# bliunlpr/Robust_e2e_gan

Measured on NVIDIA B200. Metric: utterances/sec (joint step fwd/bwd), higher is better.
Workload: dtype fp32

## Files before the change

robust_e2e_gan_b200/csrc/attloc_loop.cu:

```cuda
#include <math_constants.h>

#include "attloc_common.cuh"
#include "tc_common.cuh"

namespace re2e {
namespace {

#ifdef RE2E_ATT_DEBUG
__device__ long long g_loop_dbg[2][16 * 512];
#define LOOP_DBG_DECL                                                  \
  __shared__ long long dbg_acc[16];                                    \
  if (threadIdx.x == 0)                                                \
    for (int i_ = 0; i_ < 16; ++i_) dbg_acc[i_] = 0;                   \
  long long dbg_last = clock64()
#define LOOP_MARK(slot)                                              \
  do {                                                               \
    if (threadIdx.x == 0) {                                          \
      const long long t_ = clock64();                                \
      dbg_acc[slot] += t_ - dbg_last;                                \
      dbg_last = t_;                                                 \
    }                                                                \
  } while (0)
#define LOOP_DBG_FLUSH(which)                                                                   \
  do {                                                                                          \
    if (threadIdx.x == 0)                                                                       \
      for (int i_ = 0; i_ < 16; ++i_) g_loop_dbg[which][blockIdx.x * 16 + i_] = dbg_acc[i_];    \
  } while (0)
#else
#define LOOP_DBG_DECL
#define LOOP_MARK(slot)
#define LOOP_DBG_FLUSH(which)
#endif

__device__ __forceinline__ void cp_async4(void *dst_smem, const void *src_gmem) {
  asm volatile("cp.async.ca.shared.global [%0], [%1], 4;" ::"r"(smem_u32(dst_smem)), "l"(src_gmem) : "memory");
}
__device__ __forceinline__ void cp_async_commit() { asm volatile("cp.async.commit_group;" ::: "memory"); }
__device__ __forceinline__ void cp_async_wait_all() { asm volatile("cp.async.wait_group 0;" ::: "memory"); }

__device__ __forceinline__ void warp_reduce10(float (&v)[10], int lane) {
  {
    const bool up = lane & 16;
#pragma unroll
    for (int i = 0; i < 5; ++i) {
      const float send = up ? v[i] : v[i + 5], keep = up ? v[i + 5] : v[i];
      v[i] = keep + __shfl_xor_sync(0xffffffffu, send, 16);
    }
  }
  {
    const bool up = lane & 8;
#pragma unroll
    for (int i = 0; i < 2; ++i) {
      const float send = up ? v[i] : v[i + 3], keep = up ? v[i + 3] : v[i];
      v[i] = keep + __shfl_xor_sync(0xffffffffu, send, 8);
    }
    v[2] += __shfl_xor_sync(0xffffffffu, v[2], 8);
  }
  {
    const bool up = lane & 4;
    const float send = up ? v[0] : v[1], keep = up ? v[1] : v[0];
    v[0] = keep + __shfl_xor_sync(0xffffffffu, send, 4);
    v[2] += __shfl_xor_sync(0xffffffffu, v[2], 4);
  }
  {
    const bool up = lane & 2;
    const float send = up ? v[0] : v[2], keep = up ? v[2] : v[0];
    v[0] = keep + __shfl_xor_sync(0xffffffffu, send, 2);
  }
  v[0] += __shfl_xor_sync(0xffffffffu, v[0], 1);
}

constexpr int kLP = 8;
constexpr int kLW = 2 * kLP;
constexpr int kLT = kLW * 32;
constexpr int kLMaxCL = 8;
constexpr int kKG = 12;

struct LoopGeom {
  int tloc_max, App, CKp, Thp, Dp;
  int col_enc, ncols;
};

struct LoopFwdParams {
  const float *pre, *enc, *dec_proj, *att_init, *W_att, *W_conv, *gvec, *gvec_b;
  float scaling;
  float *c_all, *w_all, *conv_all;
  int S, B, Th, D, A, C, K;
  LoopGeom g;
};

struct LoopBwdParams {
  const float *pre, *enc, *dec_proj, *att_init, *w_all, *conv_all, *dc_all, *dw_all, *W_att, *W_conv, *gvec;
  float scaling;
  float *d_pre, *d_decproj, *acc_slots;
  int slot_stride;
  int S, B, Th, D, A, C, K;
  LoopGeom g;
};

template <int APL, int CP, int DPL>
__global__ void __launch_bounds__(kLT, 1) attloc_loop_fwd_kernel(const LoopFwdParams p) {
  constexpr int NT = kLT;
  constexpr int WP = CP + 1;
  constexpr int CPP = (CP + 3) & ~3;
  extern __shared__ __align__(128) unsigned char smraw[];
  const LoopGeom g = p.g;
  const int C = CP == 10 ? 10 : p.C;
  const int Th = p.Th, D = p.D, A = p.A, K = p.K, S = p.S, B = p.B, filts = (p.K - 1) / 2;
  const int tid = threadIdx.x, lane = tid & 31, warp = tid >> 5, half = warp & 1, pair = warp >> 1;
  const int CL = (int)cluster_nctarank(), rank = (int)cluster_ctarank();
  const int b = blockIdx.x / CL;
  const int t0 = min(Th, rank * g.tloc_max), t1 = min(Th, t0 + g.tloc_max), tloc = t1 - t0;
  const int nch = (tloc + kLP - 1) / kLP;
  const int Dp = g.Dp, Dh = (D + 1) / 2;

  uint64_t *full = reinterpret_cast<uint64_t *>(smraw);
  uint64_t *xbar = full + 1;
  uint64_t *tbar = xbar + 2;
  float *tile = reinterpret_cast<float *>(smraw + 128);
  float *app = tile + (size_t)g.tloc_max * (A + D);
  float *wc_s = app + g.App;
  float *watt_s = wc_s + g.CKp;
  float *convp = watt_s + A * WP;
  float *conv_s = convp + round4(kKQ * g.tloc_max * CP);
  float *e_all = conv_s + g.tloc_max * CPP;
  float *epart = e_all + 2 * g.Thp;
  float *cred = epart + round4(2 * g.tloc_max);
  float *cbuf = cred + kLP * Dp;

  const uint32_t xbytes = (uint32_t)Th * 4u + (rank == 0 ? (uint32_t)CL * (uint32_t)D * 4u : 0u);
  if (tid == 0) {
    mbar_init(full, 1);
    mbar_init(&xbar[0], 1);
    mbar_init(&xbar[1], 1);
    mbar_init(tbar, 1);
    mbar_fence_init();
    mbar_expect_tx(&xbar[0], xbytes);
    mbar_expect_tx(&xbar[1], xbytes);
    if (rank == 0) mbar_expect_tx(tbar, (uint32_t)CL * (uint32_t)D * 4u);
  }
  cluster_arrive_relaxed();
  float gv[APL];
#pragma unroll
  for (int j = 0; j < APL; ++j) gv[j] = __ldg(p.gvec + half * (A / 2) + lane + 32 * j);
  const float gb = __ldg(p.gvec_b);
  for (int i = tid; i < C * K; i += NT) wc_s[i] = __ldg(p.W_conv + i);
  for (int i = tid; i < A * C; i += NT) { const int a = i / C; watt_s[a * WP + (i - a * C)] = __ldg(p.W_att + i); }
  pdl_wait();
  if (tid == 0 && tloc > 0) {
    mbar_expect_tx(full, (uint32_t)tloc * (uint32_t)(A + D) * 4u);
    bulk_g2s(tile, p.pre + ((size_t)b * Th + t0) * A, (uint32_t)tloc * A * 4u, full);
    bulk_g2s(tile + (size_t)g.tloc_max * A, p.enc + ((size_t)b * Th + t0) * D, (uint32_t)tloc * D * 4u, full);
  }
  for (int i = tid; i < g.App; i += NT) {
    const int t = i - filts;
    app[i] = (t >= 0 && t < Th) ? __ldg(p.att_init + (size_t)b * Th + t) : 0.0f;
  }
  __syncthreads();
  constexpr int APH = (APL + 1) / 2;
  float2 WattP[APH][CP];
#pragma unroll
  for (int jp = 0; jp < APH; ++jp) {
    const int a0 = half * (A / 2) + lane + 32 * (2 * jp), a1 = a0 + 32;
#pragma unroll
    for (int c = 0; c < CP; ++c)
      WattP[jp][c] = make_float2(c < C ? watt_s[a0 * WP + c] : 0.0f, (c < C && 2 * jp + 1 < APL) ? watt_s[a1 * WP + c] : 0.0f);
  }
  uint32_t dmask = 0;
#pragma unroll
  for (int j = 0; j < DPL; ++j)
    if (lane + 32 * j < Dh && half * Dh + lane + 32 * j < D) dmask |= 1u << j;
  const int aoff = half * (A / 2) + lane;
  cluster_wait();
  if (tloc > 0) mbar_wait(full, 0);
  LOOP_DBG_DECL;
  LOOP_MARK(0);

  for (int s = 0; s < S; ++s) {
    const uint32_t par = (uint32_t)s & 1u, ph = ((uint32_t)s >> 1) & 1u;
    float *e_cur = e_all + par * g.Thp;
    float *cb = cbuf + par * kLMaxCL * Dp;
    float dp[APL];
#pragma unroll
    for (int j = 0; j < APL; ++j) dp[j] = __ldg(p.dec_proj + ((size_t)s * B + b) * A + aoff + 32 * j);

    {
      const int ntg = (tloc + kTG - 1) / kTG;
      const int Kq = (K + kKQ - 1) / kKQ;
      const int nitems = ntg * C * kKQ;
      for (int item = tid; item < nitems; item += NT) {
        const int tg = item % ntg, rest = item / ntg, c = rest % C, kq = rest / C;
        const int k0 = kq * Kq, k1 = min(K, k0 + Kq);
        const float *wr = wc_s + c * K;
        const float *ar = app + t0 + kTG * tg;
        float a0 = 0.f, a1 = 0.f, a2 = 0.f, a3 = 0.f, a4 = 0.f;
        float x0 = ar[k0], x1 = ar[k0 + 1], x2 = ar[k0 + 2], x3 = ar[k0 + 3];
#pragma unroll 5
        for (int k = k0; k < k1; ++k) {
          const float x4 = ar[k + 4], wv2 = wr[k];
          a0 = fmaf(wv2, x0, a0); a1 = fmaf(wv2, x1, a1); a2 = fmaf(wv2, x2, a2);
          a3 = fmaf(wv2, x3, a3); a4 = fmaf(wv2, x4, a4);
          x0 = x1; x1 = x2; x2 = x3; x3 = x4;
        }
        float *o = convp + ((size_t)kq * g.tloc_max + kTG * tg) * CP + c;
        const int nv = min(kTG, tloc - kTG * tg);
        o[0] = a0;
        if (nv > 1) o[CP] = a1;
        if (nv > 2) o[2 * CP] = a2;
        if (nv > 3) o[3 * CP] = a3;
        if (nv > 4) o[4 * CP] = a4;
      }
    }
    __syncthreads();
    LOOP_MARK(1);
    for (int i = tid; i < tloc * CPP; i += NT) {
      const int tl = i / CPP, c = i - tl * CPP;
      float v = 0.0f;
      if (c < C) {
#pragma unroll
        for (int kq = 0; kq < kKQ; ++kq) v += convp[((size_t)kq * g.tloc_max + tl) * CP + c];
        if (p.conv_all) p.conv_all[(((size_t)s * B + b) * Th + t0 + tl) * C + c] = v;
      }
      conv_s[i] = v;
    }
    __syncthreads();
    LOOP_MARK(2);

    float acc[DPL];
#pragma unroll
    for (int j = 0; j < DPL; ++j) acc[j] = 0.0f;
#pragma unroll 2
    for (int q = 0; q < nch; ++q) {
      const int tl = kLP * q + pair;
      if (tl < tloc) {
        const float *cvp = conv_s + tl * CPP;
        float cv[CPP];
#pragma unroll
        for (int c4 = 0; c4 < CPP; c4 += 4) {
          const float4 t4 = *reinterpret_cast<const float4 *>(cvp + c4);
          cv[c4] = t4.x; cv[c4 + 1] = t4.y; cv[c4 + 2] = t4.z; cv[c4 + 3] = t4.w;
        }
        const float *row = tile + (size_t)tl * A + aoff;
        const float pw = app[filts + t0 + tl];
        const float *er = tile + (size_t)g.tloc_max * A + (size_t)tl * D + half * Dh + lane;
        float part = 0.0f;
#pragma unroll
        for (int jp = 0; jp < APH; ++jp) {
          const bool two = 2 * jp + 1 < APL;
          float2 u = make_float2(dp[2 * jp] + row[64 * jp], two ? dp[2 * jp + 1] + row[64 * jp + 32] : 0.0f);
#pragma unroll
          for (int c = 0; c < CP; ++c) u = __ffma2_rn(WattP[jp][c], make_float2(cv[c], cv[c]), u);
          part = fmaf(gv[2 * jp], tanh_ex2(u.x), part);
          if (two) part = fmaf(gv[2 * jp + 1], tanh_ex2(u.y), part);
        }
#pragma unroll
        for (int j = 0; j < DPL; ++j)
          if (dmask & (1u << j)) acc[j] = fmaf(pw, er[32 * j], acc[j]);
        part = warp_sum(part);
        if (lane == 0) epart[2 * tl + half] = part;
      }
    }
#pragma unroll
    for (int j = 0; j < DPL; ++j)
      if (dmask & (1u << j)) cred[pair * Dp + half * Dh + lane + 32 * j] = acc[j];
    LOOP_MARK(3);
    __syncthreads();
    LOOP_MARK(4);

    for (int d = tid; d < D; d += NT) {
      float sum = 0.0f;
#pragma unroll
      for (int pr = 0; pr < kLP; ++pr) sum += cred[pr * Dp + d];
      st_async_f32(dsmem_addr(cb + rank * Dp + d, 0u), s > 0 ? sum : 0.0f, dsmem_addr(&xbar[par], 0u));
    }
    for (int i = tid; i < tloc * CL; i += NT) {
      const int r = i / tloc, tl = i - r * tloc;
      const float e = p.scaling * ((epart[2 * tl] + epart[2 * tl + 1]) + gb);
      st_async_f32(dsmem_addr(e_cur + t0 + tl, (uint32_t)r), e, dsmem_addr(&xbar[par], (uint32_t)r));
    }
    LOOP_MARK(5);
    mbar_wait(&xbar[par], ph);
    LOOP_MARK(6);
    float M = -CUDART_INF_F;
    for (int t = lane; t < Th; t += 32) M = fmaxf(M, e_cur[t]);
    M = warp_max(M);
    float Ssum = 0.0f;
    for (int t = lane; t < Th; t += 32) Ssum += __expf(e_cur[t] - M);
    Ssum = warp_sum(Ssum);
    const float inv = 1.0f / Ssum;
    for (int t = tid; t < Th; t += NT) {
      const float w = __expf(e_cur[t] - M) * inv;
      app[filts + t] = w;
      if (t >= t0 && t < t1) p.w_all[((size_t)s * B + b) * Th + t] = w;
    }
    if (rank == 0 && s > 0) {
      for (int d = tid; d < D; d += NT) {
        float sum = 0.0f;
        for (int r = 0; r < CL; ++r) sum += cb[r * Dp + d];
        p.c_all[((size_t)(s - 1) * B + b) * D + d] = sum;
      }
    }
    if (tid == 0) mbar_expect_tx(&xbar[par], xbytes);
    __syncthreads();
    LOOP_MARK(7);
  }
  {
    float acc[DPL];
#pragma unroll
    for (int j = 0; j < DPL; ++j) acc[j] = 0.0f;
    for (int q = 0; q < nch; ++q) {
      const int tl = kLP * q + pair;
      if (tl < tloc) {
        const float pw = app[filts + t0 + tl];
        const float *er = tile + (size_t)g.tloc_max * A + (size_t)tl * D + half * Dh + lane;
#pragma unroll
        for (int j = 0; j < DPL; ++j)
          if (dmask & (1u << j)) acc[j] = fmaf(pw, er[32 * j], acc[j]);
      }
    }
#pragma unroll
    for (int j = 0; j < DPL; ++j)
      if (dmask & (1u << j)) cred[pair * Dp + half * Dh + lane + 32 * j] = acc[j];
    __syncthreads();
    float *cb = cbuf + ((uint32_t)S & 1u) * kLMaxCL * Dp;
    for (int d = tid; d < D; d += NT) {
      float sum = 0.0f;
#pragma unroll
      for (int pr = 0; pr < kLP; ++pr) sum += cred[pr * Dp + d];
      st_async_f32(dsmem_addr(cb + rank * Dp + d, 0u), sum, dsmem_addr(tbar, 0u));
    }
    if (rank == 0) {
      mbar_wait(tbar, 0);
      for (int d = tid; d < D; d += NT) {
        float sum = 0.0f;
        for (int r = 0; r < CL; ++r) sum += cb[r * Dp + d];
        p.c_all[((size_t)(S - 1) * B + b) * D + d] = sum;
      }
    }
  }
  LOOP_DBG_FLUSH(0);
}

template <int N>
__device__ __forceinline__ void tmem_ldn(uint32_t taddr, float *v);
template <>
__device__ __forceinline__ void tmem_ldn<1>(uint32_t taddr, float *v) {
  uint32_t r0;
  asm volatile("tcgen05.ld.sync.aligned.32x32b.x1.b32 {%0}, [%1];" : "=r"(r0) : "r"(taddr));
  v[0] = __uint_as_float(r0);
}
template <>
__device__ __forceinline__ void tmem_ldn<2>(uint32_t taddr, float *v) {
  uint32_t r0, r1;
  asm volatile("tcgen05.ld.sync.aligned.32x32b.x2.b32 {%0, %1}, [%2];" : "=r"(r0), "=r"(r1) : "r"(taddr));
  v[0] = __uint_as_float(r0); v[1] = __uint_as_float(r1);
}
template <>
__device__ __forceinline__ void tmem_ldn<4>(uint32_t taddr, float *v) {
  uint32_t r0, r1, r2, r3;
  asm volatile("tcgen05.ld.sync.aligned.32x32b.x4.b32 {%0, %1, %2, %3}, [%4];"
               : "=r"(r0), "=r"(r1), "=r"(r2), "=r"(r3) : "r"(taddr));
  v[0] = __uint_as_float(r0); v[1] = __uint_as_float(r1); v[2] = __uint_as_float(r2); v[3] = __uint_as_float(r3);
}
template <>
__device__ __forceinline__ void tmem_ldn<8>(uint32_t taddr, float *v) {
  uint32_t r[8];
  asm volatile("tcgen05.ld.sync.aligned.32x32b.x8.b32 {%0, %1, %2, %3, %4, %5, %6, %7}, [%8];"
               : "=r"(r[0]), "=r"(r[1]), "=r"(r[2]), "=r"(r[3]), "=r"(r[4]), "=r"(r[5]), "=r"(r[6]), "=r"(r[7])
               : "r"(taddr));
#pragma unroll
  for (int i = 0; i < 8; ++i) v[i] = __uint_as_float(r[i]);
}
template <int N>
__device__ __forceinline__ void tmem_stn(uint32_t taddr, const float *v);
template <>
__device__ __forceinline__ void tmem_stn<1>(uint32_t taddr, const float *v) {
  asm volatile("tcgen05.st.sync.aligned.32x32b.x1.b32 [%0], {%1};" ::"r"(taddr), "r"(__float_as_uint(v[0])) : "memory");
}
template <>
__device__ __forceinline__ void tmem_stn<2>(uint32_t taddr, const float *v) {
  asm volatile("tcgen05.st.sync.aligned.32x32b.x2.b32 [%0], {%1, %2};" ::"r"(taddr), "r"(__float_as_uint(v[0])),
               "r"(__float_as_uint(v[1]))
               : "memory");
}
template <>
__device__ __forceinline__ void tmem_stn<4>(uint32_t taddr, const float *v) {
  asm volatile("tcgen05.st.sync.aligned.32x32b.x4.b32 [%0], {%1, %2, %3, %4};" ::"r"(taddr),
               "r"(__float_as_uint(v[0])), "r"(__float_as_uint(v[1])), "r"(__float_as_uint(v[2])),
               "r"(__float_as_uint(v[3]))
               : "memory");
}
template <>
__device__ __forceinline__ void tmem_stn<8>(uint32_t taddr, const float *v) {
  asm volatile("tcgen05.st.sync.aligned.32x32b.x8.b32 [%0], {%1, %2, %3, %4, %5, %6, %7, %8};" ::"r"(taddr),
               "r"(__float_as_uint(v[0])), "r"(__float_as_uint(v[1])), "r"(__float_as_uint(v[2])),
               "r"(__float_as_uint(v[3])), "r"(__float_as_uint(v[4])), "r"(__float_as_uint(v[5])),
               "r"(__float_as_uint(v[6])), "r"(__float_as_uint(v[7]))
               : "memory");
}
__device__ __forceinline__ void tmem_wait_ld() { asm volatile("tcgen05.wait::ld.sync.aligned;" ::: "memory"); }
__device__ __forceinline__ void tmem_wait_st() { asm volatile("tcgen05.wait::st.sync.aligned;" ::: "memory"); }
template <int N>
__device__ __forceinline__ void tmem_load(uint32_t taddr, float *v) {
  if constexpr (N >= 8) { tmem_ldn<8>(taddr, v); if constexpr (N > 8) tmem_load<N - 8>(taddr + 8, v + 8); }
  else if constexpr (N >= 4) { tmem_ldn<4>(taddr, v); if constexpr (N > 4) tmem_load<N - 4>(taddr + 4, v + 4); }
  else if constexpr (N >= 2) { tmem_ldn<2>(taddr, v); if constexpr (N > 2) tmem_load<N - 2>(taddr + 2, v + 2); }
  else { tmem_ldn<1>(taddr, v); }
}
template <int N>
__device__ __forceinline__ void tmem_store(uint32_t taddr, const float *v) {
  if constexpr (N >= 8) { tmem_stn<8>(taddr, v); if constexpr (N > 8) tmem_store<N - 8>(taddr + 8, v + 8); }
  else if constexpr (N >= 4) { tmem_stn<4>(taddr, v); if constexpr (N > 4) tmem_store<N - 4>(taddr + 4, v + 4); }
  else if constexpr (N >= 2) { tmem_stn<2>(taddr, v); if constexpr (N > 2) tmem_store<N - 2>(taddr + 2, v + 2); }
  else { tmem_stn<1>(taddr, v); }
}

template <int APL, int CP, int DPL2>
__global__ void __launch_bounds__(kLT, 1) attloc_loop_bwd_kernel(const LoopBwdParams p) {
  constexpr int NT = kLT;
  constexpr int WP = CP + 1;
  constexpr int CPP = (CP + 3) & ~3;
  constexpr int CH2 = (CP + 1) / 2;
  extern __shared__ __align__(128) unsigned char smraw[];
  const LoopGeom g = p.g;
  const int C = CP == 10 ? 10 : p.C;
  const int Th = p.Th, D = p.D, A = p.A, K = p.K, S = p.S, B = p.B, filts = (p.K - 1) / 2;
  const int tid = threadIdx.x, lane = tid & 31, warp = tid >> 5, half = warp & 1, pair = warp >> 1;
  const int CL = (int)cluster_nctarank(), rank = (int)cluster_ctarank();
  const int b = blockIdx.x / CL;
  const int t0 = min(Th, rank * g.tloc_max), t1 = min(Th, t0 + g.tloc_max), tloc = t1 - t0;
  const int nchx = (tloc + kLP - 1) / kLP;
  const int nche = (tloc + kLW - 1) / kLW;
  const int nchx_max = (g.tloc_max + kLP - 1) / kLP, nche_max = (g.tloc_max + kLW - 1) / kLW;

  uint64_t *done_x = reinterpret_cast<uint64_t *>(smraw);
  uint64_t *xbar1 = done_x + 1;
  uint64_t *xbar2 = xbar1 + 2;
  uint32_t *tmem_slot = reinterpret_cast<uint32_t *>(xbar2 + 2);
  float *xs = reinterpret_cast<float *>(smraw + 128);
  float *dcvT = xs + (size_t)g.tloc_max * A;
  float *app = dcvT + 2 * CP * g.App;
  float *wc_s = app + g.App;
  float *conv_s = wc_s + g.CKp;
  float *w_s = conv_s + g.tloc_max * CPP;
  float *dwt_s = w_s + round4(g.tloc_max);
  float *de_s = dwt_s + round4(g.tloc_max);
  float *dwn_s = de_s + round4(g.tloc_max);
  float *dcv_p = dwn_s + round4(g.tloc_max);
  float *ddp_w = dcv_p + 2 * g.tloc_max * 16;
  float *scr = ddp_w + kLW * (A / 2);
  float *ddp_x = scr + max(A * WP, round4(kKQ * CP * g.tloc_max));
  float *xch = ddp_x + 2 * kLMaxCL * A;
  float *slot = p.acc_slots + (size_t)blockIdx.x * p.slot_stride;

  const uint32_t x1bytes = (uint32_t)CL * 4u;
  const uint32_t x2bytes = (uint32_t)Th * (uint32_t)C * 4u + (rank == 0 ? (uint32_t)CL * (uint32_t)A * 4u : 0u);
  if (tid == 0) {
    mbar_init(done_x, kLW);
    for (int i = 0; i < 2; ++i) { mbar_init(&xbar1[i], 1); mbar_init(&xbar2[i], 1); }
    mbar_fence_init();
    for (int i = 0; i < 2; ++i) { mbar_expect_tx(&xbar1[i], x1bytes); mbar_expect_tx(&xbar2[i], x2bytes); }
  }
  cluster_arrive_relaxed();
  if (warp == 0) tmem_alloc(tmem_slot, 512);
  float gv[APL];
#pragma unroll
  for (int j = 0; j < APL; ++j) gv[j] = __ldg(p.gvec + half * (A / 2) + lane + 32 * j);
  for (int i = tid; i < C * K; i += NT) wc_s[i] = __ldg(p.W_conv + i);
  for (int i = tid; i < A * C; i += NT) { const int a = i / C; scr[a * WP + (i - a * C)] = __ldg(p.W_att + i); }
  {
    const int padn = g.App - Th;
    for (int i = tid; i < 2 * CP * padn; i += NT) {
      const int c = i / padn, o = i - c * padn;
      dcvT[c * g.App + (o < filts ? o : Th + o)] = 0.0f;
    }
    for (int i = tid; i < g.tloc_max * CPP; i += NT) conv_s[i] = 0.0f;
    for (int i = tid; i < round4(g.tloc_max); i += NT) dwn_s[i] = 0.0f;
  }
  tc_fence_before();
  __syncthreads();
  tc_fence_after();
  const uint32_t tbase = *tmem_slot + ((uint32_t)(32 * (warp & 3)) << 16);
  const uint32_t tcol_pre = tbase + (uint32_t)((warp >> 2) * nchx_max * APL);
  const uint32_t tcol_enc = tbase + (uint32_t)(g.col_enc + (warp >> 2) * nche_max * DPL2);
  float2 WattC[APL][CH2];
#pragma unroll
  for (int j = 0; j < APL; ++j) {
    const int a = half * (A / 2) + lane + 32 * j;
#pragma unroll
    for (int c2 = 0; c2 < CH2; ++c2)
      WattC[j][c2] = make_float2(2 * c2 < C ? scr[a * WP + 2 * c2] : 0.0f, 2 * c2 + 1 < C ? scr[a * WP + 2 * c2 + 1] : 0.0f);
  }
  const int aoff = half * (A / 2) + lane;
  pdl_wait();
  for (int q = 0; q < nchx; ++q) {
    const int tl = kLP * q + pair;
    float v[APL];
#pragma unroll
    for (int j = 0; j < APL; ++j) v[j] = tl < tloc ? __ldg(p.pre + ((size_t)b * Th + t0 + tl) * A + aoff + 32 * j) : 0.0f;
    tmem_store<APL>(tcol_pre + (uint32_t)(q * APL), v);
  }
  for (int q = 0; q < nche; ++q) {
    const int tl = kLW * q + warp;
    float v[DPL2];
#pragma unroll
    for (int j = 0; j < DPL2; ++j)
      v[j] = (tl < tloc && lane + 32 * j < D) ? __ldg(p.enc + ((size_t)b * Th + t0 + tl) * D + lane + 32 * j) : 0.0f;
    tmem_store<DPL2>(tcol_enc + (uint32_t)(q * DPL2), v);
  }
  tmem_wait_st();
  __syncthreads();
  cluster_wait();

  float pacc[kKG];
#pragma unroll
  for (int i = 0; i < kKG; ++i) pacc[i] = 0.0f;
  float dgv[APL];
#pragma unroll
  for (int j = 0; j < APL; ++j) dgv[j] = 0.0f;
  float dgb = 0.0f;
  const int nkg = (K + kKG - 1) / kKG;
  const bool conv_thread = tid >= A && tid - A < C * nkg;
  const int cw_c = conv_thread ? (tid - A) / nkg : 0, cw_kb = conv_thread ? ((tid - A) % nkg) * kKG : 0;
  LOOP_DBG_DECL;
  LOOP_MARK(0);

  for (int it = 0; it < S; ++it) {
    const int s = S - 1 - it;
    const uint32_t par = (uint32_t)it & 1u, ph = ((uint32_t)it >> 1) & 1u;
    float *dcv_cur = dcvT + par * CP * g.App;
    float *ddpx = ddp_x + par * kLMaxCL * A;
    float *xc = xch + par * kLMaxCL;
    const size_t sb = (size_t)s * B + b;
    float dcr[DPL2];
#pragma unroll
    for (int j = 0; j < DPL2; ++j) dcr[j] = (p.dc_all && lane + 32 * j < D) ? __ldg(p.dc_all + sb * D + lane + 32 * j) : 0.0f;
    float dp[APL];
#pragma unroll
    for (int j = 0; j < APL; ++j) dp[j] = __ldg(p.dec_proj + sb * A + aoff + 32 * j);
    for (int i = tid; i < tloc; i += NT) {
      w_s[i] = __ldg(p.w_all + sb * Th + t0 + i);
      dwt_s[i] = dwn_s[i] + (p.dw_all ? __ldg(p.dw_all + sb * Th + t0 + i) : 0.0f);
    }
    for (int i = tid; i < tloc * C; i += NT) {
      const int tl = i / C;
      conv_s[tl * CPP + (i - tl * C)] = __ldg(p.conv_all + (sb * Th + t0) * C + i);
    }
    {
      const float *prev = s == 0 ? p.att_init + (size_t)b * Th : p.w_all + (sb - B) * Th;
      for (int i = tid; i < g.App; i += NT) {
        const int t = i - filts;
        app[i] = (t >= 0 && t < Th) ? __ldg(prev + t) : 0.0f;
      }
    }
    __syncthreads();
    LOOP_MARK(1);

    for (int q = 0; q < nche; ++q) {
      const int tl = kLW * q + warp;
      float ev[DPL2];
      tmem_load<DPL2>(tcol_enc + (uint32_t)(q * DPL2), ev);
      tmem_wait_ld();
      float dot = 0.0f;
#pragma unroll
      for (int j = 0; j < DPL2; ++j) dot = fmaf(dcr[j], ev[j], dot);
      dot = warp_sum(dot);
      if (lane == 0 && tl < tloc) dwt_s[tl] += dot;
    }
    __syncthreads();
    LOOP_MARK(2);
    if (warp == 0) {
      float s1 = 0.0f;
      for (int tl = lane; tl < tloc; tl += 32) s1 = fmaf(w_s[tl], dwt_s[tl], s1);
      s1 = warp_sum(s1);
      if (lane < CL) st_async_f32(dsmem_addr(xc + rank, (uint32_t)lane), s1, dsmem_addr(&xbar1[par], (uint32_t)lane));
    }
    mbar_wait(&xbar1[par], ph);
    float Stot = 0.0f;
    for (int r = 0; r < CL; ++r) Stot += xc[r];
    for (int tl = tid; tl < tloc; tl += NT) de_s[tl] = p.scaling * w_s[tl] * (dwt_s[tl] - Stot);
    if (tid == 0) {
      mbar_expect_tx(&xbar1[par], x1bytes);
      if (it > 0) bulk_wait<0>();
    }
    __syncthreads();
    LOOP_MARK(3);

    float ddp[APL];
#pragma unroll
    for (int j = 0; j < APL; ++j) ddp[j] = 0.0f;
    float pn[APL];
    tmem_load<APL>(tcol_pre, pn);
#pragma unroll 1
    for (int q = 0; q < nchx; ++q) {
      const int tl = kLP * q + pair;
      tmem_wait_ld();
      float pv[APL];
#pragma unroll
      for (int j = 0; j < APL; ++j) {
        asm volatile("" : "+f"(pn[j]));
        pv[j] = pn[j];
      }
      if (q + 1 < nchx) tmem_load<APL>(tcol_pre + (uint32_t)((q + 1) * APL), pn);
      if (tl < tloc) {
        const float de = de_s[tl];
        const float *cvp = conv_s + tl * CPP;
        float cv[CPP];
#pragma unroll
        for (int c4 = 0; c4 < CPP; c4 += 4) {
          const float4 t4 = *reinterpret_cast<const float4 *>(cvp + c4);
          cv[c4] = t4.x; cv[c4 + 1] = t4.y; cv[c4 + 2] = t4.z; cv[c4 + 3] = t4.w;
        }
        float2 dcv2[8];
#pragma unroll
        for (int c = 0; c < 8; ++c) dcv2[c] = make_float2(0.0f, 0.0f);
        float *row = xs + (size_t)tl * A + aoff;
#pragma unroll
        for (int j = 0; j < APL; ++j) {
          float2 u2 = make_float2(pv[j] + dp[j], 0.0f);
#pragma unroll
          for (int c2 = 0; c2 < CH2; ++c2)
            u2 = __ffma2_rn(WattC[j][c2], make_float2(cv[2 * c2], 2 * c2 + 1 < CPP ? cv[2 * c2 + 1] : 0.0f), u2);
          const float x = tanh_ex2(u2.x + u2.y);
          dgv[j] = fmaf(de, x, dgv[j]);
          const float dt = de * gv[j] * (1.0f - x * x);
          ddp[j] += dt;
          row[32 * j] = dt;
          const float2 dt2 = make_float2(dt, dt);
#pragma unroll
          for (int c2 = 0; c2 < CH2; ++c2) dcv2[c2] = __ffma2_rn(dt2, WattC[j][c2], dcv2[c2]);
        }
        if constexpr (CP == 10) {
          float dcv[10];
#pragma unroll
          for (int c = 0; c < 5; ++c) { dcv[2 * c] = dcv2[c].x; dcv[2 * c + 1] = dcv2[c].y; }
          warp_reduce10(dcv, lane);
          if ((lane & 1) == 0 && ((lane & 2) == 0 || (lane & 12) == 0)) {
            const int b4 = (lane >> 4) & 1, b3 = (lane >> 3) & 1, b2 = (lane >> 2) & 1;
            const int ci = 5 * b4 + ((lane & 2) ? 2 : (b2 ? (b3 ? 4 : 1) : (b3 ? 3 : 0)));
            dcv_p[(half * g.tloc_max + tl) * 16 + ci] = dcv[0];
          }
        } else {
          float dcv[16];
#pragma unroll
          for (int c = 0; c < 8; ++c) { dcv[2 * c] = dcv2[c].x; dcv[2 * c + 1] = dcv2[c].y; }
          warp_reduce16(dcv, lane);
          if ((lane & 1) == 0) {
            const int ci = ((lane >> 4) & 1) * 8 + ((lane >> 3) & 1) * 4 + ((lane >> 2) & 1) * 2 + ((lane >> 1) & 1);
            dcv_p[(half * g.tloc_max + tl) * 16 + ci] = dcv[0];
          }
// ... 91 lines not shown
#pragma unroll 5
        for (int k = k0; k < k1; ++k) {
          const float x0 = dr[-k], wv = wr[k];
          a0 = fmaf(wv, x0, a0); a1 = fmaf(wv, x1, a1); a2 = fmaf(wv, x2, a2);
          a3 = fmaf(wv, x3, a3); a4 = fmaf(wv, x4, a4);
          x4 = x3; x3 = x2; x2 = x1; x1 = x0;
        }
        float *o = scr + ((size_t)(kq * C + c)) * g.tloc_max + kTG * sg;
        const int nv = min(kTG, tloc - kTG * sg);
        o[0] = a0;
        if (nv > 1) o[1] = a1;
        if (nv > 2) o[2] = a2;
        if (nv > 3) o[3] = a3;
        if (nv > 4) o[4] = a4;
      }
    }
    if (tid == 0) mbar_expect_tx(&xbar2[par], x2bytes);
    __syncthreads();
    LOOP_MARK(9);
    if (s > 0) {
      for (int tl = tid; tl < tloc; tl += NT) {
        float sum = 0.0f;
        for (int i = 0; i < kKQ * C; ++i) sum += scr[(size_t)i * g.tloc_max + tl];
        dwn_s[tl] = sum;
      }
    }
    LOOP_MARK(10);
  }

  LOOP_DBG_FLUSH(1);
  if (tid < A) {
#pragma unroll
    for (int c = 0; c < CP; ++c)
      if (c < C) slot[tid * C + c] = pacc[c];
  } else if (conv_thread) {
#pragma unroll
    for (int i = 0; i < kKG; ++i)
      if (cw_kb + i < K) slot[A * C + cw_c * K + cw_kb + i] = pacc[i];
  }
  __syncthreads();
#pragma unroll
  for (int j = 0; j < APL; ++j) ddp_w[warp * (A / 2) + lane + 32 * j] = dgv[j];
  __syncthreads();
  for (int a = tid; a < A; a += NT) {
    const int h = a >= A / 2 ? 1 : 0, ai = a - h * (A / 2);
    float sg = 0.0f;
#pragma unroll
    for (int pr = 0; pr < kLP; ++pr) sg += ddp_w[(2 * pr + h) * (A / 2) + ai];
    slot[A * C + C * K + a] = sg;
  }
  if (warp == kLW - 1 && lane == 0) slot[A * C + C * K + A] = dgb;
  if (tid == 0) bulk_wait<0>();
  tc_fence_before();
  __syncthreads();
  if (warp == 0) tmem_dealloc(*tmem_slot, 512);
}

inline int loop_check_dims(int S, int B, int Th, int D, int A, int C, int K) {
  if (S <= 0 || B <= 0 || Th <= 0 || D <= 0 || A <= 0 || C <= 0 || K <= 0) return RE2E_E_ARG;
  if ((K & 1) == 0) return RE2E_E_ARG;
  if (A % 64 != 0 || A > 512 || (D & 3) || D > 512 || C > 16) return RE2E_E_UNSUPPORTED;
  const int apl = A / 64;
  if (!(apl == 1 || apl == 2 || apl == 4 || apl == 5 || apl == 8)) return RE2E_E_UNSUPPORTED;
  return RE2E_OK;
}

inline int pick_cl(int B, int Th) {
  const int sms = num_sms();
  int CL = 1;
  while (CL < kLMaxCL && B * CL * 2 <= sms) CL *= 2;
  while (CL > 1 && (Th + CL - 1) / CL < kLP) CL /= 2;
  return CL;
}

inline void loop_geom_common(int Th, int D, int C, int K, int CL, LoopGeom &g) {
  const int filts = (K - 1) / 2;
  g.tloc_max = (Th + CL - 1) / CL;
  g.App = round4(Th + 2 * filts + 8);
  g.CKp = round4(C * K);
  g.Thp = round4(Th);
  g.Dp = round4(D);
  g.col_enc = 0;
  g.ncols = 0;
}

inline bool loop_geom_fwd(int B, int Th, int D, int A, int C, int K, int CP, int &CL, LoopGeom &g, size_t &smem) {
  CL = pick_cl(B, Th);
  const int CPP = round4(CP);
  for (;;) {
    loop_geom_common(Th, D, C, K, CL, g);
    const size_t floats = (size_t)g.tloc_max * (A + D) + g.App + g.CKp + (size_t)A * (CP + 1) +
                          round4(kKQ * g.tloc_max * CP) + (size_t)g.tloc_max * CPP + 2 * (size_t)g.Thp +
                          round4(g.tloc_max) + round4(2 * g.tloc_max) + 2 * kLW + (size_t)kLP * g.Dp +
                          2 * (size_t)kLMaxCL * g.Dp + 4 * kLMaxCL;
    smem = 128 + sizeof(float) * floats;
    if (smem <= 226 * 1024) return true;
    if (CL >= kLMaxCL || B * CL * 2 > num_sms()) return false;
    CL *= 2;
  }
}

inline bool loop_geom_bwd(int B, int Th, int D, int A, int C, int K, int CP, int dpl2, int &CL, LoopGeom &g,
                          size_t &smem) {
  CL = pick_cl(B, Th);
  const int CPP = round4(CP);
  const int nkg = (K + kKG - 1) / kKG;
  if (A + C * nkg > kLT) return false;
  for (;;) {
    loop_geom_common(Th, D, C, K, CL, g);
    const int nchx_max = (g.tloc_max + kLP - 1) / kLP, nche_max = (g.tloc_max + kLW - 1) / kLW;
    g.col_enc = 4 * nchx_max * (A / 64);
    g.ncols = g.col_enc + 4 * nche_max * dpl2;
    const size_t scr = (size_t)A * (CP + 1) > (size_t)round4(kKQ * CP * g.tloc_max) ? (size_t)A * (CP + 1)
                                                                                   : (size_t)round4(kKQ * CP * g.tloc_max);
    const size_t floats = (size_t)g.tloc_max * A + 2 * (size_t)CP * g.App + g.App + g.CKp + (size_t)g.tloc_max * CPP +
                          4 * (size_t)round4(g.tloc_max) + 2 * (size_t)g.tloc_max * 16 + (size_t)kLW * (A / 2) + scr +
                          2 * (size_t)kLMaxCL * A + 2 * kLMaxCL;
    smem = 128 + sizeof(float) * floats;
    if (smem <= 226 * 1024 && g.ncols <= 512) return true;
    if (CL >= kLMaxCL || B * CL * 2 > num_sms()) return false;
    CL *= 2;
  }
}

template <typename Kern, typename Params>
int launch_loop(Kern kern, const Params &prm, int B, int CL, size_t smem, cudaStream_t st) {
  int rc0 = ensure_smem(reinterpret_cast<const void *>(kern), smem);
  if (rc0 != RE2E_OK) return rc0;
  cudaLaunchConfig_t cfg{};
  cfg.gridDim = dim3((unsigned)(B * CL));
  cfg.blockDim = dim3((unsigned)kLT);
  cfg.dynamicSmemBytes = smem;
  cfg.stream = st;
  cudaLaunchAttribute attr[2];
  attr[0].id = cudaLaunchAttributeClusterDimension;
  attr[0].val.clusterDim.x = (unsigned)CL;
  attr[0].val.clusterDim.y = 1;
  attr[0].val.clusterDim.z = 1;
  attr[1].id = cudaLaunchAttributeProgrammaticStreamSerialization;
  attr[1].val.programmaticStreamSerializationAllowed = 1;
  cfg.attrs = attr;
  cfg.numAttrs = 2;
  cudaError_t e = cudaLaunchKernelEx(&cfg, kern, prm);
  count_launch();
  return e == cudaSuccess ? RE2E_OK : (int)e;
}

#define LOOP_DISPATCH(NAME, APLV, CPV, ...)                                             \
  switch (APLV) {                                                                       \
    case 1: rc = (CPV) == 10 ? NAME<1, 10> __VA_ARGS__ : NAME<1, 16> __VA_ARGS__; break; \
    case 2: rc = (CPV) == 10 ? NAME<2, 10> __VA_ARGS__ : NAME<2, 16> __VA_ARGS__; break; \
    case 4: rc = (CPV) == 10 ? NAME<4, 10> __VA_ARGS__ : NAME<4, 16> __VA_ARGS__; break; \
    case 5: rc = (CPV) == 10 ? NAME<5, 10> __VA_ARGS__ : NAME<5, 16> __VA_ARGS__; break; \
    case 8: rc = (CPV) == 10 ? NAME<8, 10> __VA_ARGS__ : NAME<8, 16> __VA_ARGS__; break; \
    default: rc = RE2E_E_UNSUPPORTED;                                                   \
  }

template <int APL, int CP>
int run_loop_fwd(const LoopFwdParams &prm, int CL, size_t smem, cudaStream_t st) {
  if (prm.D == prm.A) return launch_loop(attloc_loop_fwd_kernel<APL, CP, APL>, prm, prm.B, CL, smem, st);
  return launch_loop(attloc_loop_fwd_kernel<APL, CP, 8>, prm, prm.B, CL, smem, st);
}
template <int APL, int CP>
int run_loop_bwd(const LoopBwdParams &prm, int CL, size_t smem, cudaStream_t st) {
  if (prm.D == prm.A) return launch_loop(attloc_loop_bwd_kernel<APL, CP, 2 * APL>, prm, prm.B, CL, smem, st);
  return launch_loop(attloc_loop_bwd_kernel<APL, CP, 16>, prm, prm.B, CL, smem, st);
}

}
}

using namespace re2e;

#ifdef RE2E_ATT_DEBUG
extern "C" int re2e_loop_debug_read(long long *host_out, int which) {
  cudaDeviceSynchronize();
  return (int)cudaMemcpyFromSymbol(host_out, g_loop_dbg, sizeof(long long) * 16 * 512, sizeof(long long) * 16 * 512 * which);
}
#endif

extern "C" int re2e_attloc_loop_supported(int S, int B, int Th, int D, int A, int C, int K) {
  int rc = loop_check_dims(S, B, Th, D, A, C, K);
  if (rc != RE2E_OK) return 0;
  const int CP = C == 10 ? 10 : 16;
  int CLf, CLb;
  size_t smem;
  LoopGeom g;
  if (!loop_geom_fwd(B, Th, D, A, C, K, CP, CLf, g, smem)) return 0;
  if (!loop_geom_bwd(B, Th, D, A, C, K, CP, D == A ? 2 * (A / 64) : 16, CLb, g, smem)) return 0;
  return 1;
}

extern "C" int re2e_attloc_loop_slots(int S, int B, int Th, int D, int A, int C, int K) {
  int rc = loop_check_dims(S, B, Th, D, A, C, K);
  if (rc != RE2E_OK) return rc;
  int CL;
  size_t smem;
  LoopGeom g;
  if (!loop_geom_bwd(B, Th, D, A, C, K, C == 10 ? 10 : 16, D == A ? 2 * (A / 64) : 16, CL, g, smem))
    return RE2E_E_UNSUPPORTED;
  return B * CL;
}

extern "C" int re2e_attloc_loop_fwd(const float *pre, const float *enc_h, const float *dec_proj,
                                    const float *att_init, const float *W_att, const float *W_conv,
                                    const float *gvec, const float *gvec_b, float scaling, float *c_all,
                                    float *w_all, float *conv_all, int S, int B, int Th, int D, int A, int C,
                                    int K, void *stream) {
  RE2E_CHECK_ARG(pre && enc_h && dec_proj && att_init && W_att && W_conv && gvec && gvec_b && c_all && w_all);
  int rc = loop_check_dims(S, B, Th, D, A, C, K);
  if (rc != RE2E_OK) return rc;
  RE2E_CHECK_ARG(aligned16(pre) && aligned16(enc_h));
  const int CP = C == 10 ? 10 : 16;
  LoopFwdParams prm;
  prm.pre = pre; prm.enc = enc_h; prm.dec_proj = dec_proj; prm.att_init = att_init; prm.W_att = W_att;
  prm.W_conv = W_conv; prm.gvec = gvec; prm.gvec_b = gvec_b; prm.scaling = scaling; prm.c_all = c_all;
  prm.w_all = w_all; prm.conv_all = conv_all;
  prm.S = S; prm.B = B; prm.Th = Th; prm.D = D; prm.A = A; prm.C = C; prm.K = K;
  int CL;
  size_t smem;
  if (!loop_geom_fwd(B, Th, D, A, C, K, CP, CL, prm.g, smem)) return RE2E_E_UNSUPPORTED;
  LOOP_DISPATCH(run_loop_fwd, A / 64, CP, (prm, CL, smem, static_cast<cudaStream_t>(stream)));
  return rc;
}

extern "C" int re2e_attloc_loop_bwd(const float *pre, const float *enc_h, const float *dec_proj,
                                    const float *att_init, const float *w_all, const float *conv_all,
                                    const float *dc_all, const float *dw_all, const float *W_att,
                                    const float *W_conv, const float *gvec, float scaling, float *d_pre,
                                    float *d_decproj, float *acc_slots, int n_slots, int S, int B, int Th, int D,
                                    int A, int C, int K, void *stream) {
  RE2E_CHECK_ARG(pre && enc_h && dec_proj && att_init && w_all && conv_all && W_att && W_conv && gvec);
  RE2E_CHECK_ARG(d_pre && d_decproj && acc_slots);
  int rc = loop_check_dims(S, B, Th, D, A, C, K);
  if (rc != RE2E_OK) return rc;
  RE2E_CHECK_ARG(aligned16(d_pre));
  const int CP = C == 10 ? 10 : 16;
  LoopBwdParams prm;
  prm.pre = pre; prm.enc = enc_h; prm.dec_proj = dec_proj; prm.att_init = att_init; prm.w_all = w_all;
  prm.conv_all = conv_all; prm.dc_all = dc_all; prm.dw_all = dw_all; prm.W_att = W_att; prm.W_conv = W_conv;
  prm.gvec = gvec; prm.scaling = scaling; prm.d_pre = d_pre; prm.d_decproj = d_decproj; prm.acc_slots = acc_slots;
  prm.slot_stride = (int)re2e_attloc_acc_floats(A, C, K);
  prm.S = S; prm.B = B; prm.Th = Th; prm.D = D; prm.A = A; prm.C = C; prm.K = K;
  int CL;
  size_t smem;
  if (!loop_geom_bwd(B, Th, D, A, C, K, CP, D == A ? 2 * (A / 64) : 16, CL, prm.g, smem)) return RE2E_E_UNSUPPORTED;
  if (n_slots < B * CL) return RE2E_E_WORKSPACE;
  LOOP_DISPATCH(run_loop_bwd, A / 64, CP, (prm, CL, smem, static_cast<cudaStream_t>(stream)));
  return rc;
}
```

Measured before the change: 24830.

## Batch attention-context products out of the serial step loop into chunked epilogues

```diff
diff --git a/robust_e2e_gan_b200/csrc/attloc_loop.cu b/robust_e2e_gan_b200/csrc/attloc_loop.cu
--- a/robust_e2e_gan_b200/csrc/attloc_loop.cu
+++ b/robust_e2e_gan_b200/csrc/attloc_loop.cu
@@ -75,10 +75,14 @@
 constexpr int kLT = kLW * 32;
 constexpr int kLMaxCL = 8;
 constexpr int kKG = 12;
+constexpr int kSCMax = 64;
+constexpr int kRSF = 4;
+constexpr int kDJ = 5;
 
 struct LoopGeom {
   int tloc_max, App, CKp, Thp, Dp;
   int col_enc, ncols;
+  int sc;
 };
 
 struct LoopFwdParams {
@@ -98,7 +102,7 @@
   LoopGeom g;
 };
 
-template <int APL, int CP, int DPL>
+template <int APL, int CP>
 __global__ void __launch_bounds__(kLT, 1) attloc_loop_fwd_kernel(const LoopFwdParams p) {
   constexpr int NT = kLT;
   constexpr int WP = CP + 1;
@@ -112,11 +116,9 @@
   const int b = blockIdx.x / CL;
   const int t0 = min(Th, rank * g.tloc_max), t1 = min(Th, t0 + g.tloc_max), tloc = t1 - t0;
   const int nch = (tloc + kLP - 1) / kLP;
-  const int Dp = g.Dp, Dh = (D + 1) / 2;
 
   uint64_t *full = reinterpret_cast<uint64_t *>(smraw);
   uint64_t *xbar = full + 1;
-  uint64_t *tbar = xbar + 2;
   float *tile = reinterpret_cast<float *>(smraw + 128);
   float *app = tile + (size_t)g.tloc_max * (A + D);
   float *wc_s = app + g.App;
@@ -125,19 +127,18 @@
   float *conv_s = convp + round4(kKQ * g.tloc_max * CP);
   float *e_all = conv_s + g.tloc_max * CPP;
   float *epart = e_all + 2 * g.Thp;
-  float *cred = epart + round4(2 * g.tloc_max);
-  float *cbuf = cred + kLP * Dp;
-
-  const uint32_t xbytes = (uint32_t)Th * 4u + (rank == 0 ? (uint32_t)CL * (uint32_t)D * 4u : 0u);
+  const int scp = round4(g.sc);
+  float *wT = watt_s;
+  float *Pc = wT + (size_t)g.tloc_max * scp;
+
+  const uint32_t xbytes = (uint32_t)Th * 4u;
   if (tid == 0) {
     mbar_init(full, 1);
     mbar_init(&xbar[0], 1);
     mbar_init(&xbar[1], 1);
-    mbar_init(tbar, 1);
     mbar_fence_init();
     mbar_expect_tx(&xbar[0], xbytes);
     mbar_expect_tx(&xbar[1], xbytes);
-    if (rank == 0) mbar_expect_tx(tbar, (uint32_t)CL * (uint32_t)D * 4u);
   }
   cluster_arrive_relaxed();
   float gv[APL];
@@ -166,10 +167,6 @@
     for (int c = 0; c < CP; ++c)
       WattP[jp][c] = make_float2(c < C ? watt_s[a0 * WP + c] : 0.0f, (c < C && 2 * jp + 1 < APL) ? watt_s[a1 * WP + c] : 0.0f);
   }
-  uint32_t dmask = 0;
-#pragma unroll
-  for (int j = 0; j < DPL; ++j)
-    if (lane + 32 * j < Dh && half * Dh + lane + 32 * j < D) dmask |= 1u << j;
   const int aoff = half * (A / 2) + lane;
   cluster_wait();
   if (tloc > 0) mbar_wait(full, 0);
@@ -179,7 +176,6 @@
   for (int s = 0; s < S; ++s) {
     const uint32_t par = (uint32_t)s & 1u, ph = ((uint32_t)s >> 1) & 1u;
     float *e_cur = e_all + par * g.Thp;
-    float *cb = cbuf + par * kLMaxCL * Dp;
     float dp[APL];
 #pragma unroll
     for (int j = 0; j < APL; ++j) dp[j] = __ldg(p.dec_proj + ((size_t)s * B + b) * A + aoff + 32 * j);
@@ -226,9 +222,6 @@
     __syncthreads();
     LOOP_MARK(2);
 
-    float acc[DPL];
-#pragma unroll
-    for (int j = 0; j < DPL; ++j) acc[j] = 0.0f;
 #pragma unroll 2
     for (int q = 0; q < nch; ++q) {
       const int tl = kLP * q + pair;
@@ -241,8 +234,6 @@
           cv[c4] = t4.x; cv[c4 + 1] = t4.y; cv[c4 + 2] = t4.z; cv[c4 + 3] = t4.w;
         }
         const float *row = tile + (size_t)tl * A + aoff;
-        const float pw = app[filts + t0 + tl];
-        const float *er = tile + (size_t)g.tloc_max * A + (size_t)tl * D + half * Dh + lane;
         float part = 0.0f;
 #pragma unroll
         for (int jp = 0; jp < APH; ++jp) {
@@ -253,26 +244,14 @@
           part = fmaf(gv[2 * jp], tanh_ex2(u.x), part);
           if (two) part = fmaf(gv[2 * jp + 1], tanh_ex2(u.y), part);
         }
-#pragma unroll
-        for (int j = 0; j < DPL; ++j)
-          if (dmask & (1u << j)) acc[j] = fmaf(pw, er[32 * j], acc[j]);
         part = warp_sum(part);
         if (lane == 0) epart[2 * tl + half] = part;
       }
     }
-#pragma unroll
-    for (int j = 0; j < DPL; ++j)
-      if (dmask & (1u << j)) cred[pair * Dp + half * Dh + lane + 32 * j] = acc[j];
     LOOP_MARK(3);
     __syncthreads();
     LOOP_MARK(4);
 
-    for (int d = tid; d < D; d += NT) {
-      float sum = 0.0f;
-#pragma unroll
-      for (int pr = 0; pr < kLP; ++pr) sum += cred[pr * Dp + d];
-      st_async_f32(dsmem_addr(cb + rank * Dp + d, 0u), s > 0 ? sum : 0.0f, dsmem_addr(&xbar[par], 0u));
-    }
     for (int i = tid; i < tloc * CL; i += NT) {
       const int r = i / tloc, tl = i - r * tloc;
       const float e = p.scaling * ((epart[2 * tl] + epart[2 * tl + 1]) + gb);
@@ -293,51 +272,71 @@
       app[filts + t] = w;
       if (t >= t0 && t < t1) p.w_all[((size_t)s * B + b) * Th + t] = w;
     }
-    if (rank == 0 && s > 0) {
-      for (int d = tid; d < D; d += NT) {
-        float sum = 0.0f;
-        for (int r = 0; r < CL; ++r) sum += cb[r * Dp + d];
-        p.c_all[((size_t)(s - 1) * B + b) * D + d] = sum;
-      }
-    }
     if (tid == 0) mbar_expect_tx(&xbar[par], xbytes);
     __syncthreads();
     LOOP_MARK(7);
   }
   {
-    float acc[DPL];
-#pragma unroll
-    for (int j = 0; j < DPL; ++j) acc[j] = 0.0f;
-    for (int q = 0; q < nch; ++q) {
-      const int tl = kLP * q + pair;
-      if (tl < tloc) {
-        const float pw = app[filts + t0 + tl];
-        const float *er = tile + (size_t)g.tloc_max * A + (size_t)tl * D + half * Dh + lane;
-#pragma unroll
-        for (int j = 0; j < DPL; ++j)
-          if (dmask & (1u << j)) acc[j] = fmaf(pw, er[32 * j], acc[j]);
-      }
-    }
-#pragma unroll
-    for (int j = 0; j < DPL; ++j)
-      if (dmask & (1u << j)) cred[pair * Dp + half * Dh + lane + 32 * j] = acc[j];
-    __syncthreads();
-    float *cb = cbuf + ((uint32_t)S & 1u) * kLMaxCL * Dp;
-    for (int d = tid; d < D; d += NT) {
-      float sum = 0.0f;
-#pragma unroll
-      for (int pr = 0; pr < kLP; ++pr) sum += cred[pr * Dp + d];
-      st_async_f32(dsmem_addr(cb + rank * Dp + d, 0u), sum, dsmem_addr(tbar, 0u));
-    }
-    if (rank == 0) {
-      mbar_wait(tbar, 0);
-      for (int d = tid; d < D; d += NT) {
+    const float *encs = tile + (size_t)g.tloc_max * A;
+    const int ncg = (D + 32 * kDJ - 1) / (32 * kDJ);
+    const int dsl = round4((D + CL - 1) / CL);
+    for (int s0 = 0; s0 < S; s0 += g.sc) {
+      const int nsc = min(g.sc, S - s0);
+      if (s0 > 0) cluster_sync_all();
+      for (int i = tid; i < tloc * nsc; i += NT) {
+        const int j = i / tloc, tl = i - j * tloc;
+        wT[tl * scp + j] = p.w_all[((size_t)(s0 + j) * B + b) * Th + t0 + tl];
+      }
+      __syncthreads();
+      const int nsg = (nsc + kRSF - 1) / kRSF;
+      for (int task = warp; task < nsg * ncg; task += kLW) {
+        const int j0 = kRSF * (task % nsg), d0 = 32 * kDJ * (task / nsg) + lane;
+        float tot[kRSF][kDJ];
+#pragma unroll
+        for (int r = 0; r < kRSF; ++r)
+#pragma unroll
+          for (int q = 0; q < kDJ; ++q) tot[r][q] = 0.0f;
+#pragma unroll 1
+        for (int pr = 0; pr < kLP; ++pr) {
+          float acc[kRSF][kDJ];
+#pragma unroll
+          for (int r = 0; r < kRSF; ++r)
+#pragma unroll
+            for (int q = 0; q < kDJ; ++q) acc[r][q] = 0.0f;
+#pragma unroll 1
+          for (int tl = pr; tl < tloc; tl += kLP) {
+            const float4 w4 = *reinterpret_cast<const float4 *>(wT + tl * scp + j0);
+            const float wv[kRSF] = {w4.x, w4.y, w4.z, w4.w};
+#pragma unroll
+            for (int q = 0; q < kDJ; ++q) {
+              const float e = d0 + 32 * q < D ? encs[(size_t)tl * D + d0 + 32 * q] : 0.0f;
+#pragma unroll
+              for (int r = 0; r < kRSF; ++r) acc[r][q] = fmaf(wv[r], e, acc[r][q]);
+            }
+          }
+#pragma unroll
+          for (int r = 0; r < kRSF; ++r)
+#pragma unroll
+            for (int q = 0; q < kDJ; ++q) tot[r][q] += acc[r][q];
+        }
+#pragma unroll
+        for (int r = 0; r < kRSF; ++r)
+#pragma unroll
+          for (int q = 0; q < kDJ; ++q)
+            if (j0 + r < nsc && d0 + 32 * q < D) Pc[(size_t)(j0 + r) * g.Dp + d0 + 32 * q] = tot[r][q];
+      }
+      cluster_sync_all();
+      const int dlo = rank * dsl, dn = max(0, min(D, dlo + dsl) - dlo);
+      for (int i = tid; i < nsc * dn; i += NT) {
+        const int j = i / dn, d = dlo + (i - j * dn);
         float sum = 0.0f;
-        for (int r = 0; r < CL; ++r) sum += cb[r * Dp + d];
-        p.c_all[((size_t)(S - 1) * B + b) * D + d] = sum;
-      }
-    }
-  }
+        for (int r = 0; r < CL; ++r) sum += dsmem_ld(dsmem_addr(Pc + (size_t)j * g.Dp + d, (uint32_t)r));
+        p.c_all[((size_t)(s0 + j) * B + b) * D + d] = sum;
+      }
+    }
+    cluster_sync_all();
+  }
+  LOOP_MARK(8);
   LOOP_DBG_FLUSH(0);
 }
 
@@ -432,6 +431,7 @@
   const int nchx = (tloc + kLP - 1) / kLP;
   const int nche = (tloc + kLW - 1) / kLW;
   const int nchx_max = (g.tloc_max + kLP - 1) / kLP, nche_max = (g.tloc_max + kLW - 1) / kLW;
+  const int tlp = round4(g.tloc_max);
 
   uint64_t *done_x = reinterpret_cast<uint64_t *>(smraw);
   uint64_t *xbar1 = done_x + 1;
@@ -443,8 +443,8 @@
   float *wc_s = app + g.App;
   float *conv_s = wc_s + g.CKp;
   float *w_s = conv_s + g.tloc_max * CPP;
-  float *dwt_s = w_s + round4(g.tloc_max);
-  float *de_s = dwt_s + round4(g.tloc_max);
+  float *dwx = w_s + tlp;
+  float *de_s = dwx + (size_t)g.sc * tlp;
   float *dwn_s = de_s + round4(g.tloc_max);
   float *dcv_p = dwn_s + round4(g.tloc_max);
   float *ddp_w = dcv_p + 2 * g.tloc_max * 16;
@@ -532,15 +532,41 @@
     float *ddpx = ddp_x + par * kLMaxCL * A;
     float *xc = xch + par * kLMaxCL;
     const size_t sb = (size_t)s * B + b;
-    float dcr[DPL2];
-#pragma unroll
-    for (int j = 0; j < DPL2; ++j) dcr[j] = (p.dc_all && lane + 32 * j < D) ? __ldg(p.dc_all + sb * D + lane + 32 * j) : 0.0f;
+    if (it % g.sc == 0) {
+      const int nsc = min(g.sc, S - it);
+      if (p.dc_all == nullptr) {
+        for (int i = tid; i < nsc * tlp; i += NT) dwx[i] = 0.0f;
+      } else {
+#pragma unroll 1
+        for (int i = 0; i < nsc; ++i) {
+          const float *dcrow = p.dc_all + ((size_t)(S - 1 - it - i) * B + b) * D;
+          float dcr[DPL2];
+#pragma unroll
+          for (int j = 0; j < DPL2; ++j) dcr[j] = lane + 32 * j < D ? __ldg(dcrow + lane + 32 * j) : 0.0f;
+#pragma unroll 1
+          for (int q = 0; q < nche; ++q) {
+            const int tl = kLW * q + warp;
+            float ev[DPL2];
+            tmem_load<DPL2>(tcol_enc + (uint32_t)(q * DPL2), ev);
+            tmem_wait_ld();
+            float dot = 0.0f;
+#pragma unroll
+            for (int j = 0; j < DPL2; ++j) dot = fmaf(dcr[j], ev[j], dot);
+            dot = warp_sum(dot);
+            if (lane == 0 && tl < tloc) dwx[(size_t)i * tlp + tl] = dot;
+          }
+        }
+      }
+      __syncthreads();
+    }
+    float *dwt_s = dwx + (size_t)(it % g.sc) * tlp;
+    LOOP_MARK(1);
     float dp[APL];
 #pragma unroll
     for (int j = 0; j < APL; ++j) dp[j] = __ldg(p.dec_proj + sb * A + aoff + 32 * j);
     for (int i = tid; i < tloc; i += NT) {
       w_s[i] = __ldg(p.w_all + sb * Th + t0 + i);
-      dwt_s[i] = dwn_s[i] + (p.dw_all ? __ldg(p.dw_all + sb * Th + t0 + i) : 0.0f);
+      dwt_s[i] = (dwn_s[i] + (p.dw_all ? __ldg(p.dw_all + sb * Th + t0 + i) : 0.0f)) + dwt_s[i];
     }
     for (int i = tid; i < tloc * C; i += NT) {
       const int tl = i / C;
@@ -552,20 +578,6 @@
         const int t = i - filts;
         app[i] = (t >= 0 && t < Th) ? __ldg(prev + t) : 0.0f;
       }
-    }
-    __syncthreads();
-    LOOP_MARK(1);
-
-    for (int q = 0; q < nche; ++q) {
-      const int tl = kLW * q + warp;
-      float ev[DPL2];
-      tmem_load<DPL2>(tcol_enc + (uint32_t)(q * DPL2), ev);
-      tmem_wait_ld();
-      float dot = 0.0f;
-#pragma unroll
-      for (int j = 0; j < DPL2; ++j) dot = fmaf(dcr[j], ev[j], dot);
-      dot = warp_sum(dot);
-      if (lane == 0 && tl < tloc) dwt_s[tl] += dot;
     }
     __syncthreads();
     LOOP_MARK(2);
@@ -823,25 +835,30 @@
   g.Dp = round4(D);
   g.col_enc = 0;
   g.ncols = 0;
-}
-
-inline bool loop_geom_fwd(int B, int Th, int D, int A, int C, int K, int CP, int &CL, LoopGeom &g, size_t &smem) {
+  g.sc = 1;
+}
+
+inline bool loop_geom_fwd(int S, int B, int Th, int D, int A, int C, int K, int CP, int &CL, LoopGeom &g,
+                          size_t &smem) {
   CL = pick_cl(B, Th);
   const int CPP = round4(CP);
   for (;;) {
     loop_geom_common(Th, D, C, K, CL, g);
-    const size_t floats = (size_t)g.tloc_max * (A + D) + g.App + g.CKp + (size_t)A * (CP + 1) +
-                          round4(kKQ * g.tloc_max * CP) + (size_t)g.tloc_max * CPP + 2 * (size_t)g.Thp +
-                          round4(g.tloc_max) + round4(2 * g.tloc_max) + 2 * kLW + (size_t)kLP * g.Dp +
-                          2 * (size_t)kLMaxCL * g.Dp + 4 * kLMaxCL;
-    smem = 128 + sizeof(float) * floats;
+    const size_t steps = (size_t)A * (CP + 1) + round4(kKQ * g.tloc_max * CP) + (size_t)g.tloc_max * CPP +
+                         2 * (size_t)g.Thp + round4(2 * g.tloc_max);
+    const size_t fixed = (size_t)g.tloc_max * (A + D) + g.App + g.CKp + round4(g.tloc_max) + 2 * kLW + 4 * kLMaxCL;
+    for (g.sc = std::min(S, kSCMax);; --g.sc) {
+      const size_t epi = (size_t)g.tloc_max * round4(g.sc) + (size_t)g.sc * g.Dp;
+      smem = 128 + sizeof(float) * (fixed + std::max(steps, epi));
+      if (smem <= 226 * 1024 || g.sc == 1) break;
+    }
     if (smem <= 226 * 1024) return true;
     if (CL >= kLMaxCL || B * CL * 2 > num_sms()) return false;
     CL *= 2;
   }
 }
 
-inline bool loop_geom_bwd(int B, int Th, int D, int A, int C, int K, int CP, int dpl2, int &CL, LoopGeom &g,
+inline bool loop_geom_bwd(int S, int B, int Th, int D, int A, int C, int K, int CP, int dpl2, int &CL, LoopGeom &g,
                           size_t &smem) {
   CL = pick_cl(B, Th);
   const int CPP = round4(CP);
@@ -855,10 +872,15 @@
     const size_t scr = (size_t)A * (CP + 1) > (size_t)round4(kKQ * CP * g.tloc_max) ? (size_t)A * (CP + 1)
                                                                                    : (size_t)round4(kKQ * CP * g.tloc_max);
     const size_t floats = (size_t)g.tloc_max * A + 2 * (size_t)CP * g.App + g.App + g.CKp + (size_t)g.tloc_max * CPP +
-                          4 * (size_t)round4(g.tloc_max) + 2 * (size_t)g.tloc_max * 16 + (size_t)kLW * (A / 2) + scr +
+                          3 * (size_t)round4(g.tloc_max) + 2 * (size_t)g.tloc_max * 16 + (size_t)kLW * (A / 2) + scr +
                           2 * (size_t)kLMaxCL * A + 2 * kLMaxCL;
+    const size_t row = sizeof(float) * (size_t)round4(g.tloc_max);
     smem = 128 + sizeof(float) * floats;
-    if (smem <= 226 * 1024 && g.ncols <= 512) return true;
+    if (smem + row <= 226 * 1024 && g.ncols <= 512) {
+      g.sc = (int)std::min<size_t>((size_t)std::min(S, kSCMax), (226 * 1024 - smem) / row);
+      smem += row * g.sc;
+      return true;
+    }
     if (CL >= kLMaxCL || B * CL * 2 > num_sms()) return false;
     CL *= 2;
   }
@@ -899,8 +921,7 @@
 
 template <int APL, int CP>
 int run_loop_fwd(const LoopFwdParams &prm, int CL, size_t smem, cudaStream_t st) {
-  if (prm.D == prm.A) return launch_loop(attloc_loop_fwd_kernel<APL, CP, APL>, prm, prm.B, CL, smem, st);
-  return launch_loop(attloc_loop_fwd_kernel<APL, CP, 8>, prm, prm.B, CL, smem, st);
+  return launch_loop(attloc_loop_fwd_kernel<APL, CP>, prm, prm.B, CL, smem, st);
 }
 template <int APL, int CP>
 int run_loop_bwd(const LoopBwdParams &prm, int CL, size_t smem, cudaStream_t st) {
@@ -927,8 +948,8 @@
   int CLf, CLb;
   size_t smem;
   LoopGeom g;
-  if (!loop_geom_fwd(B, Th, D, A, C, K, CP, CLf, g, smem)) return 0;
-  if (!loop_geom_bwd(B, Th, D, A, C, K, CP, D == A ? 2 * (A / 64) : 16, CLb, g, smem)) return 0;
+  if (!loop_geom_fwd(S, B, Th, D, A, C, K, CP, CLf, g, smem)) return 0;
+  if (!loop_geom_bwd(S, B, Th, D, A, C, K, CP, D == A ? 2 * (A / 64) : 16, CLb, g, smem)) return 0;
   return 1;
 }
 
@@ -938,7 +959,7 @@
   int CL;
   size_t smem;
   LoopGeom g;
-  if (!loop_geom_bwd(B, Th, D, A, C, K, C == 10 ? 10 : 16, D == A ? 2 * (A / 64) : 16, CL, g, smem))
+  if (!loop_geom_bwd(S, B, Th, D, A, C, K, C == 10 ? 10 : 16, D == A ? 2 * (A / 64) : 16, CL, g, smem))
     return RE2E_E_UNSUPPORTED;
   return B * CL;
 }
@@ -960,7 +981,7 @@
   prm.S = S; prm.B = B; prm.Th = Th; prm.D = D; prm.A = A; prm.C = C; prm.K = K;
   int CL;
   size_t smem;
-  if (!loop_geom_fwd(B, Th, D, A, C, K, CP, CL, prm.g, smem)) return RE2E_E_UNSUPPORTED;
+  if (!loop_geom_fwd(S, B, Th, D, A, C, K, CP, CL, prm.g, smem)) return RE2E_E_UNSUPPORTED;
   LOOP_DISPATCH(run_loop_fwd, A / 64, CP, (prm, CL, smem, static_cast<cudaStream_t>(stream)));
   return rc;
 }
@@ -985,7 +1006,7 @@
   prm.S = S; prm.B = B; prm.Th = Th; prm.D = D; prm.A = A; prm.C = C; prm.K = K;
   int CL;
   size_t smem;
-  if (!loop_geom_bwd(B, Th, D, A, C, K, CP, D == A ? 2 * (A / 64) : 16, CL, prm.g, smem)) return RE2E_E_UNSUPPORTED;
+  if (!loop_geom_bwd(S, B, Th, D, A, C, K, CP, D == A ? 2 * (A / 64) : 16, CL, prm.g, smem)) return RE2E_E_UNSUPPORTED;
   if (n_slots < B * CL) return RE2E_E_WORKSPACE;
   LOOP_DISPATCH(run_loop_bwd, A / 64, CP, (prm, CL, smem, static_cast<cudaStream_t>(stream)));
   return rc;
```

Result: slower. 24400 (median of 6 runs) (-1.7%).
